# uncbiag/DeepAtlas

Measured on AMD Instinct MI355X. Metric: training volumes/sec at 160x192x160 fp32; Dice vs CPU ref, higher is better.
Workload: dtype f32; 1 GPU; seg-only UNet_light + softmax-Dice + Adam training step, batch 2/GPU, 160x192x160 fp32 (BASELINE configs[1]); global_batch=2, n_classes=32, parallelism=dp1, matrix_precision=fp32_split, hip_graph=False, matrix_arithmetic_bits=22

## Files before the change

### __graft_entry__.py

```python
import os
import subprocess
import sys

ROOT = os.path.dirname(os.path.abspath(__file__))
CSRC = os.path.join(ROOT, 'deepatlas_amd', 'csrc')
LIB = os.path.join(CSRC, 'libdeepatlas_hip.so')
HIP_SOURCES = ['norm_act.hip', 'pool.hip', 'warp.hip', 'losses.hip', 'headdice.hip', 'xent.hip', 'reglosses.hip', 'mi.hip', 'datapath.hip', 'conv3d.hip', 'conv3d_mfma.hip', 'conv3d_flow.hip', 'conv3d_flowmm.hip', 'conv3d_s2.hip', 'conv3d_s2n.hip', 'conv3d_up2.hip', 'deconv.hip', 'pointwise_mfma.hip', 'optim.hip', 'augment.hip', 'regeval.hip', 'jacpen.hip', 'invcons.hip', 'affine.hip', 'fieldinv.hip', 'cc.hip', 'edt.hip', 'intensity.hip']


def _newer(target, deps):
    if not os.path.isfile(target):
        return True
    t = os.path.getmtime(target)
    return any(os.path.getmtime(d) > t for d in deps)


def build(force=False):
    srcs = [os.path.join(CSRC, s) for s in HIP_SOURCES]
    deps = srcs + [os.path.join(CSRC, 'common.h'), os.path.join(CSRC, 'conv3d_internal.h'), os.path.join(CSRC, 'split_f16.h'), os.path.join(CSRC, 'pointwise_internal.h'), os.path.join(CSRC, 'conv3d_wgring.h'), os.path.join(CSRC, 'conv3d_stage.h'), os.path.join(CSRC, 'bspline.h'), os.path.join(CSRC, 'counter_hash.h'),
                   os.path.join(ROOT, 'include', 'deepatlas_hip.h')]
    if force or _newer(LIB, deps):
        hipcc = os.environ.get('HIPCC', '/opt/rocm/bin/hipcc')
        objs = []
        procs = []
        for s in srcs:
            o = s[:-4] + '.o'
            objs.append(o)
            if force or _newer(o, [s] + deps[len(srcs):]):
                procs.append((s, subprocess.Popen([hipcc, '--offload-arch=gfx950', '-O3', '-std=c++17', '-fPIC', '-c', s, '-o', o])))
        for s, p in procs:
            if p.wait() != 0:
                raise RuntimeError('hipcc failed on %s' % s)
        subprocess.check_call([hipcc, '--offload-arch=gfx950', '-shared', '-fPIC'] + objs + ['-o', LIB])
    prim = os.path.join(ROOT, 'oracle', 'prim.c')
    prim_so = os.path.join(ROOT, 'oracle', 'libprim.so')
    if os.path.isfile(prim) and (force or _newer(prim_so, [prim])):
        subprocess.check_call(['gcc', '-O2', '-fPIC', '-shared', '-std=c99', prim, '-lm', '-o', prim_so])
    if ROOT not in sys.path:
        sys.path.insert(0, ROOT)
    import deepatlas_amd
    from deepatlas_amd import _native
    _native.lib()
    return LIB


def build_asan(sources=None, opt='-O1'):
    hipcc = os.environ.get('HIPCC', '/opt/rocm/bin/hipcc')
    out_dir = os.path.join(CSRC, 'asan')
    os.makedirs(out_dir, exist_ok=True)
    names = list(sources) if sources else HIP_SOURCES
    flags = ['--offload-arch=gfx950', '-fsanitize=address', '-fno-gpu-sanitize', '-shared-libsan', '-g', opt, '-std=c++17', '-fPIC']
    procs, objs = [], []
# ... 91 lines not shown
```

### deepatlas_amd/_native.py

```python
import ctypes
import os
from ctypes import c_int, c_float, c_double, c_longlong, c_size_t, c_void_p, c_char_p, POINTER

import torch

_HERE = os.path.dirname(os.path.abspath(__file__))
LIB_PATH = os.environ.get('DA_LIB') or os.path.join(_HERE, 'csrc', 'libdeepatlas_hip.so')

P = c_void_p
I = c_int
F = c_float
LL = c_longlong
SZ = c_size_t
DBL = c_double

SIGNATURES = {
    'da_version': (I, []),
    'da_device_info': (I, [POINTER(c_int), POINTER(c_int), POINTER(c_size_t), c_char_p, I]),
    'da_w_oik_to_tio': (I, [P, P, I, I, I, P]),
    'da_w_tio_to_oik': (I, [P, P, I, I, I, P]),
    'da_w_iok_to_tio': (I, [P, P, I, I, I, P]),
    'da_w_tio_to_iok': (I, [P, P, I, I, I, P]),
    'da_w_iok_flip_to_tio': (I, [P, P, I, I, I, P]),
    'da_w_tio_to_iok_flip': (I, [P, P, I, I, I, P]),
    'da_w_tio_to_oik_acc': (I, [P, P, I, I, I, P]),
    'da_w_tio_to_iok_acc': (I, [P, P, I, I, I, P]),
    'da_w_tio_to_iok_flip_acc': (I, [P, P, I, I, I, P]),
    'da_conv3d_k3_ws_bytes': (SZ, [I, I, I, I, I, I, I]),
    'da_conv3d_k3_pack_bytes': (SZ, [I, I, I, I, I, I]),
    'da_conv3d_k3_dgrad_bst': (I, [P, P, P, I, P, I, I, I, I, I, I, P, P, F, P, I, P, P, SZ, P]),
    'da_conv3d_k3_prepack': (I, [P, I, I, I, I, I, I, I, I, P, SZ, P, SZ, P, P]),
    'da_conv3d_k3_use_prepacked': (None, [P, P, SZ, P, SZ]),
    'da_conv3d_k3_prepack_many': (I, [I, P, P, P, P, P, P, P, P, P, P, P, P, P, P, P]),
    'da_conv3d_k3_fwd': (I, [P, I, P, I, P, P, P, I, I, I, I, I, I, F, P, SZ, P]),
    'da_conv3d_k3_fwd_bnstats': (I, [P, I, P, I, P, P, P, I, I, I, I, I, I, P, I, POINTER(c_int), P, SZ, P]),
    'da_conv3d_k3_dgrad': (I, [P, P, P, I, P, I, I, I, I, I, I, I, P, SZ, P]),
    'da_conv3d_k3_wgrad': (I, [P, I, P, I, P, P, P, I, I, I, I, I, I, P, SZ, P]),
    'da_conv3d_k3_fwd_pro': (I, [P, I, P, P, F, P, I, P, P, F, P, P, P, I, I, I, I, I, F, P, I, POINTER(c_int), P, SZ, P]),
    'da_conv3d_k3_wgrad_pro': (I, [P, I, P, P, F, P, I, P, P, F, P, P, I, I, I, I, I, P, SZ, P]),
    'da_upconv3d_k3_supported': (I, [I, I, I]),
    'da_upconv3d_k3_ws_bytes': (SZ, [I, I, I, I, I, I]),
    'da_upconv3d_k3_fwd': (I, [P, I, P, I, P, P, P, I, I, I, I, I, F, P, SZ, P]),
    'da_upconv3d_k3_dgrad': (I, [P, P, P, I, P, I, I, I, I, I, I, P, SZ, P]),
    'da_upconv3d_k3_wgrad': (I, [P, I, P, I, P, P, I, I, I, I, I, P, SZ, P]),
    'da_set_conv_direct': (I, [I]),
    'da_set_matrix_bf16': (I, [I]),
    'da_set_matrix_mode': (I, [I]),
    'da_pointwise_ws_bytes': (SZ, [I, I, I]),
    'da_conv1x1_fwd': (I, [P, P, P, P, LL, I, I, P, SZ, P]),
    'da_conv1x1_fwd_pro': (I, [P, P, P, F, P, P, P, LL, I, I, P, SZ, P]),
    'da_conv1x1_wgrad_pro': (I, [P, P, P, F, P, P, P, LL, I, I, P, SZ, P]),
    'da_conv1x1_dgrad': (I, [P, P, P, LL, I, I, P, SZ, P]),
    'da_conv1x1_wgrad_ws_bytes': (SZ, [LL, I, I]),
    'da_conv1x1_wgrad': (I, [P, P, P, P, LL, I, I, P, SZ, P]),
    'da_deconv_k2s2_fwd': (I, [P, P, P, P, I, I, I, I, I, I, P, SZ, P]),
    'da_deconv_k2s2_fwd_bnstats': (I, [P, P, P, P, I, I, I, I, I, I, P, I, POINTER(c_int), P, SZ, P]),
    'da_deconv_k2s2_dgrad': (I, [P, P, P, I, I, I, I, I, I, P, SZ, P]),
    'da_deconv_k2s2_bn_bwd_ws_bytes': (SZ, [I, I, I, I, I, I]),
    'da_deconv_k2s2_bn_bwd': (I, [P, P, P, P, P, P, F, P, P, P, P, P, P, P, I, I, I, I, I, I, P, I, P, SZ, P]),
    'da_deconv_k2s2_wgrad_ws_bytes': (SZ, [I, I, I, I, I, I]),
    'da_deconv_k2s2_wgrad': (I, [P, P, P, P, I, I, I, I, I, I, P, SZ, P]),
    'da_bn_ws_bytes': (SZ, [LL, I]),
    'da_bn_train_stats': (I, [P, LL, I, P, P, F, F, P, P, P, P, P, P, P, SZ, P]),
# ... 251 lines not shown
```

### deepatlas_amd/csrc/conv3d_mfma.hip

```cpp
#include "common.h"
#include "conv3d_internal.h"
#include "split_f16.h"

#include "conv3d_stage.h"

namespace {


template <int CK, int NREP, bool MASKED = false, int STATS = 0, bool BF = false, bool PRO = false, bool SP = false, int S2F = 0, bool PAIR = false, bool HB = false>
__global__ void __launch_bounds__(256, 2) conv3_mfma_fwd_kernel(FwdP p) {
    static_assert(!HB || (BF && !SP), "bf16 activation storage: bf16 matrix mode only");
    static_assert(STATS != 2 || (SP && NREP == 1 && !PRO), "BatchNorm-backward sums: the split mode's one-N-tile data gradient");
    static_assert((S2F != 0) == MASKED, "the tap-masked (stride-2) variants and only they address X / dX through the space-to-depth view");
    static_assert(!PAIR || (SP && NREP == 1 && !PRO), "paired staging: split mode, one N-tile, no input prologue");
    static_assert(!SP || (BF && !MASKED && CK == 8), "split mode: dense bf16 K = 32 kernels on 8-channel chunks");
    constexpr int NP = SP ? 2 : 1;
    constexpr bool RAW = HB && BF && !SP && !PRO && !MASKED && S2F == 0;
    extern __shared__ __attribute__((aligned(16))) float lds[];
    constexpr bool K32 = BF && !MASKED;
    using AElem = std::conditional_t<BF, short, float>;
    using Frag = std::conditional_t<SP, f16x8, std::conditional_t<K32, bf16x8, std::conditional_t<BF, s16x4, f32x4>>>;
    constexpr int EB = BF ? 2 : 4;
    constexpr int TZ = 4, HZ = TZ + 2;
    constexpr int NSTEPS = K32 ? (CK == 16 ? 14 : 7) : (27 * CK + 15) / 16;
// ... 1284 lines not shown
                acc[c][d][0] += v.x; acc[c][d][1] += v.y; acc[c][d][2] += v.z; acc[c][d][3] += v.w;
            }
    };
    if (wave >= 2) put(wave - 2);
    __syncthreads();
    if (wave < 2) add(wave);
    __syncthreads();
    if (wave == 1) put(0);
    __syncthreads();
    if (wave == 0) {
        add(0);
        float* part = p.partial + (size_t)slab * p.O;
        const int Cin = p.C1 + p.C2;
        const int co = cg * CG + i;
#pragma unroll
        for (int c = 0; c < 5; ++c)
#pragma unroll
            for (int d = 0; d < 3; ++d)
#pragma unroll
                for (int reg = 0; reg < 4; ++reg) {
                    const int row = 4 * g + reg;
                    const int combo = c < 4 ? 2 * c + (row >> 3) : 8;
                    const int dyt = c < 4 ? d : 2 * d + (row >> 3);
                    const int tap = (combo / 3) * 9 + dyt * 3 + combo % 3, ci = row & 7;
                    if (dyt < 3 && (c < 4 || d < 2) && co < p.Cout) part[((size_t)tap * Cin + cbase + ci) * p.Cout + co] = acc[c][d][reg];
                }
    }
}

#ifndef DA_WG16_ZPAD
#define DA_WG16_ZPAD 4
#endif
#include "conv3d_wgring.h"

__global__ void slab_reduce_kernel(const float* __restrict__ partial, int nparts, int O, float* __restrict__ out) {
    for (int o = blockIdx.x * blockDim.x + threadIdx.x; o < O; o += gridDim.x * blockDim.x) {
        double s = 0.0;
        for (int b = 0; b < nparts; ++b) s += (double)partial[(size_t)b * O + o];
        out[o] = (float)s;
    }
}

struct ScP {
    const float* in1; const float* in2; int C1, C2;
    const float* dy; float* partial;
    int N, D, H, W, Cout; long long nrows;
    const float* dyb; int Cd1;
};

template <int MT, int NT>
__global__ void __launch_bounds__(256) conv3_smallcin_wgrad_kernel(ScP p) {
    __shared__ __attribute__((aligned(16))) float red[MT * NT * 64 * 4];
    const int lane = threadIdx.x & 63;
    const int wave = threadIdx.x >> 6;
    const int i = lane & 15, g = lane >> 4;
    const int Cin = p.C1 + p.C2;
    int dz[MT], dy_[MT], dx[MT], cs[MT], cc[MT]; bool mval[MT]; const float* src[MT];
#pragma unroll
    for (int mt = 0; mt < MT; ++mt) {
        const int m = 16 * mt + i;
        mval[mt] = m < 27 * Cin;
        const int tap = mval[mt] ? m / Cin : 0, ci = mval[mt] ? m % Cin : 0;
        dz[mt] = tap / 9 - 1; dy_[mt] = (tap / 3) % 3 - 1; dx[mt] = tap % 3 - 1;
        if (ci < p.C1) { src[mt] = p.in1; cs[mt] = p.C1; cc[mt] = ci; } else { src[mt] = p.in2; cs[mt] = p.C2; cc[mt] = ci - p.C1; }
    }
    f32x4 acc[MT][NT];
// ... 221 lines not shown
    { static int occ = -1; if (occ < 0) { occ = getenv("DA_OCC") ? 1 : 0; if (occ) { int nb = 0; (void)hipOccupancyMaxActiveBlocksPerMultiprocessor(&nb, kern, 256, shm); fprintf(stderr, "[occ] <%d,%d,M%d,S%d,BF%d,PRO%d,SP%d> lds %zu B -> %d workgroups per CU\n", CK, NREP, (int)MASKED, (int)STATS, (int)BF, (int)PRO, (int)SP, shm, nb); } } }
    if (want) {
        unsigned long long h[6]; (void)hipStreamSynchronize(st); (void)hipMemcpy(h, dclk, 48, hipMemcpyDeviceToHost);
        fprintf(stderr, "[clk] cycles %llu realtime %llu -> %.0f MHz; grid %d x %d: starts span %.1f us, ends span %.1f us, first start -> last end %.1f us\n", h[0], h[1],
                (double)h[0] / (double)h[1] * 100.0, p.nblocks, gy, (h[3] - h[2]) * 0.01, (h[5] - h[4]) * 0.01, (h[5] - h[2]) * 0.01);
        if (getenv("DA_CLK_DUMP")) {
            static unsigned long long rec[2048];
            const int nb = p.nblocks < 1024 ? p.nblocks : 1024;
            (void)hipMemcpy(rec, dclk + 8, (size_t)nb * 16, hipMemcpyDeviceToHost);
            for (int b = 0; b < nb; ++b) fprintf(stderr, "[blk] %d xcc %llu hwid %08llx life_us %.1f\n", b, (rec[2 * b] >> 32) & 15, rec[2 * b] & 0xffffffffull, rec[2 * b + 1] * 0.01);
        }
    }
    return 0;
}

template <int CK, int NREP, unsigned F>
static int launch_fwd_prec(bool bf, bool hb, const FwdP& p, int gy, hipStream_t st) {
    return hb ? launch_fwd_mfma<CK, NREP, F | kHb>(p, gy, st) : bf ? launch_fwd_mfma<CK, NREP, F | kBf16>(p, gy, st) : launch_fwd_mfma<CK, NREP, F>(p, gy, st);
}
template <unsigned F>
static int launch_fwd_dense(int CK, int NREP, bool bf, bool hb, const FwdP& p, int gy, hipStream_t st) {
    if (CK == 16 && NREP == 1) return launch_fwd_prec<16, 1, F>(bf, hb, p, gy, st);
    if (CK == 16 && NREP == 2) return launch_fwd_prec<16, 2, F>(bf, hb, p, gy, st);
    if (CK == 8 && NREP == 1) return launch_fwd_prec<8, 1, F>(bf, hb, p, gy, st);
    if (CK == 8 && NREP == 2) return launch_fwd_prec<8, 2, F>(bf, hb, p, gy, st);
    return DA_ERR_UNSUPPORTED;
}
template <int NREP>
static int launch_fwd_split(bool stats, bool pro, const FwdP& p, int gy, hipStream_t st) {
    return stats ? (pro ? launch_fwd_mfma<8, NREP, kSplit | kStats | kPro>(p, gy, st) : launch_fwd_mfma<8, NREP, kSplit | kStats>(p, gy, st))
                 : (pro ? launch_fwd_mfma<8, NREP, kSplit | kPro>(p, gy, st) : launch_fwd_mfma<8, NREP, kSplit>(p, gy, st));
}

static const int kProMaxC = 2048;
static int pro_identity(const float** ones, const float** zeros) {
    static float* buf = nullptr;
    if (!buf) {
        hipError_t e = hipMalloc(&buf, 2 * kProMaxC * sizeof(float));
        if (e != hipSuccess) return (int)e;
        float* h = (float*)malloc(2 * kProMaxC * sizeof(float));
        for (int i = 0; i < kProMaxC; ++i) { h[i] = 1.f; h[kProMaxC + i] = 0.f; }
        e = hipMemcpy(buf, h, 2 * kProMaxC * sizeof(float), hipMemcpyHostToDevice);
        free(h);
        if (e != hipSuccess) return (int)e;
    }
    *ones = buf; *zeros = buf + kProMaxC;
    return 0;
}

template <typename P>
static int set_prologue(P& p, const DaPro* pro, int C2) {
    p.ps1 = p.pt1 = p.ps2 = p.pt2 = nullptr; p.pslope1 = p.pslope2 = -1.f;
    if (!pro) return 0;
    const float *ones, *zeros;
    if (const int rc = pro_identity(&ones, &zeros)) return rc;
    const float a = pro->s1 ? pro->slope1 : -1.f, b = (C2 > 0 && pro->s2) ? pro->slope2 : -1.f;
    if (a >= 1.f || b >= 1.f) return DA_ERR_UNSUPPORTED;
    p.pslope1 = a < 0.f ? 1.f : a; p.pslope2 = b < 0.f ? 1.f : b;
    p.ps1 = pro->s1 ? pro->s1 : ones; p.pt1 = pro->s1 ? pro->t1 : zeros;
    p.ps2 = (C2 > 0 && pro->s2) ? pro->s2 : ones; p.pt2 = (C2 > 0 && pro->s2) ? pro->t2 : zeros;
    return 0;
}

enum FwdFamily { kFamDense, kFamMasked, kFamSplit, kFamPaired, kFamBst };
struct FwdPlan {
    bool split, bf; int CK, NREP, gy, NTpad;
    int pkmode, NSTEPS;
    size_t pk, tt;
    int ntz, nty, ntx, ntiles, nblocks; FwdFamily family;
};
static int fwd_plan(const ConvGemm& c, int mode, FwdPlan* plan) {
    FwdPlan& q = *plan;
    const int Cin = c.C1 + c.C2;
    q.CK = pick_ck(c.C1, c.C2);
    if (!q.CK) return DA_ERR_UNSUPPORTED;
    if (c.pro && (c.s2d_cin > 0 || c.flipped_tr || Cin > kProMaxC)) return DA_ERR_UNSUPPORTED;
    if (c.s2d_cin > 0 && !c.s2f) return DA_ERR_UNSUPPORTED;
    q.split = mode == 2 && c.s2d_cin == 0;
    q.bf = mode == 1;
    if (q.split) q.CK = 8;
    {
        const int cin = c.C1 > c.C2 ? c.C1 : c.C2, cs = c.Cs1 > c.Cs2 ? c.Cs1 : c.Cs2;
        if ((unsigned long long)c.D * c.H * c.W * 4ull * (unsigned long long)(cin > cs ? cin : cs) >= 0xFFFFFFF0ull) return DA_ERR_UNSUPPORTED;
    }
    const int NT = (c.Cout + 15) / 16;
    q.NREP = pick_nrep(NT);
    if ((q.bf || q.split || c.pro) && q.NREP > 2) q.NREP = 2;
    if (c.s2d_cin > 0 && q.NREP > 2) q.NREP = 2;
    const bool want_bst = c.bst.y != nullptr && q.split && c.stats_partial != nullptr;
    if (want_bst) q.NREP = 1;
    q.ntz = (c.D + 3) / 4; q.nty = (c.H + TY - 1) / TY; q.ntx = (c.W + TX - 1) / TX;
    q.ntiles = c.N * q.ntz * q.nty * q.ntx;
    if (c.s2d_cin == 0 && q.NREP > 1 && !want_bst) {
        const long long tiles = (long long)c.N * q.ntz * q.nty * q.ntx;
        auto cost = [&](int nrep) {
            const int g = (NT + nrep - 1) / nrep;
            long long nb = 512 / g; if (nb < 1) nb = 1; if (nb > tiles) nb = tiles;
            return (double)((tiles + nb - 1) / nb) * nrep * (nrep == 1 ? 1.08 : 1.0);
        };
        if (cost(1) < cost(q.NREP)) q.NREP = 1;
    }
    q.gy = (NT + q.NREP - 1) / q.NREP; q.NTpad = q.gy * q.NREP;
    q.pkmode = q.split ? 3 : q.bf ? (c.s2d_cin > 0 ? 1 : 2) : 0;
    q.NSTEPS = q.pkmode >= 2 ? (q.CK == 16 ? 14 : 7) : (27 * q.CK + 15) / 16;
    q.pk = packed_bytes(Cin, c.Cout, q.CK); q.tt = tile_table_bytes(c.N, c.D, c.H, c.W);
    q.nblocks = 512 / q.gy; if (q.nblocks < 1) q.nblocks = 1; if (q.nblocks > q.ntiles) q.nblocks = q.ntiles;
    if (q.nblocks >= 8) q.nblocks &= ~7;
    if (!q.split) q.family = c.s2d_cin > 0 ? kFamMasked : kFamDense;
    else if (want_bst) q.family = kFamBst;
    else q.family = (q.NREP == 1 && !c.pro && c.C1 % 16 == 0 && c.C2 % 16 == 0) ? kFamPaired : kFamSplit;
    if (q.family == kFamMasked && q.CK != 16) return DA_ERR_UNSUPPORTED;
    if (q.family == kFamBst && (c.pro || c.Cs2 != 0 || q.gy > 2)) return DA_ERR_UNSUPPORTED;
    return 0;
}

static int fwd_launches(const ConvGemm& c, int mode, ConvGemm l[2]) {
    l[0] = c;
    if (!(mode == 2 && c.flipped_tr && c.s2d_cin == 0 && (!c.stats_partial || c.bst.y) && !c.pro && c.Cs1 == 32 && c.Cs2 == 16 && c.Cout == 48 &&
          pick_ck(c.C1, c.C2) != 0)) return 1;
    l[0].out2 = nullptr; l[0].Cs2 = 0; l[0].Cout = 32; l[0].CoutW = 48; l[0].pack = ConvPack{{c.pack.buf[0], nullptr}, {c.pack.bytes[0], 0}};
    l[1] = l[0];
    l[1].bias = c.bias ? c.bias + 32 : nullptr; l[1].out1 = c.out2; l[1].Cs1 = 16; l[1].Cout = 16; l[1].cout0 = 32;
    l[1].stats_partial = nullptr; l[1].stats_nparts = nullptr; l[1].bst = ConvBst{}; l[1].pack = ConvPack{{c.pack.buf[1], nullptr}, {c.pack.bytes[1], 0}};
    return 2;
}

static PackJob pack_job(const ConvGemm& c, const FwdPlan& q, char* base) {
    return PackJob{c.w_tio, reinterpret_cast<unsigned short*>(base), reinterpret_cast<int*>(base + q.pk - da_align(kWexpInts * sizeof(int))), reinterpret_cast<int4*>(base + q.pk),
                   c.C1 + c.C2, c.Cout, q.NTpad, c.flipped_tr, q.ntiles, q.ntx, q.nty, q.ntz, c.cout0, c.CoutW ? c.CoutW : c.Cout};
}
static void launch_split_pack(const PackJob& j, hipStream_t st) {
    hipLaunchKernelGGL(pack_split_weights_kernel, dim3(j.Cin / 8, 8), dim3(256), 0, st, j.w, j.wp, j.wexp, j.Cin, j.Cout, j.NTpad, j.flipped, j.tiles, j.ntiles, j.ntx, j.nty, j.ntz, j.cout0, j.CoutW);
}

struct Handover { const float* w; ConvPack pack; };
static thread_local Handover g_handover = {nullptr, {}};
static ConvPack take_handover(const float* w_tio) {
    const Handover h = g_handover;
    g_handover = Handover{nullptr, {}};
    return h.w == w_tio ? h.pack : ConvPack{};
}

static int conv3_mfma_launch(const ConvGemm& c) {
    FwdPlan q;
    if (const int rc = fwd_plan(c, da_matrix_mode(), &q)) return rc;
    const int Cin = c.C1 + c.C2, CK = q.CK, NREP = q.NREP, gy = q.gy;
    const bool bf = q.bf, hb = c.act_bf16 != 0, stats = c.stats_partial != nullptr, pro = c.pro != nullptr;
    hipStream_t st = c.st;
    const bool kept = q.split && c.pack.buf[0] && c.pack.bytes[0] >= q.pk + q.tt;
    if (!kept && c.ws_bytes < q.pk + q.tt) return DA_ERR_WS_SMALL;
    if (q.split && Cin / 8 > kWexpInts) return DA_ERR_UNSUPPORTED;
    const PackJob j = pack_job(c, q, kept ? reinterpret_cast<char*>(const_cast<void*>(c.pack.buf[0])) : reinterpret_cast<char*>(c.ws));
    const long long total = (long long)(Cin / CK) * q.NSTEPS * q.NTpad * 256;
    if (!q.split)
        hipLaunchKernelGGL(pack_fwd_weights_kernel, dim3(da_grid(total > q.ntiles ? total : q.ntiles, 256, 1024)), dim3(256), 0, st, c.w_tio, reinterpret_cast<float*>(j.wp), Cin, c.Cout, CK, q.NSTEPS, q.NTpad,
                           c.flipped_tr, total, q.pkmode, j.tiles, q.ntiles, q.ntx, q.nty, q.ntz, j.cout0, j.CoutW);
    else if (!kept) launch_split_pack(j, st);
    DA_LAUNCH_CHECK();
    FwdP p;
    const bool bst = q.family == kFamBst;
    p.bst_y = bst ? c.bst.y : nullptr; p.bst_par = bst ? c.bst.par : nullptr; p.bst_slope = bst ? c.bst.slope : -1.f;
    p.tiles = j.tiles; p.wp = reinterpret_cast<float*>(j.wp); p.wexp = j.wexp;
    p.in1 = c.in1; p.in2 = c.in2; p.C1 = c.C1; p.C2 = c.C2; p.bias = c.bias;
    p.out1 = c.out1; p.out2 = c.out2; p.Cs1 = c.Cs1; p.Cs2 = c.Cs2;
    p.N = c.N; p.D = c.D; p.H = c.H; p.W = c.W; p.Cout = c.Cout; p.NT = q.NTpad;
    p.ntz = q.ntz; p.nty = q.nty; p.ntx = q.ntx; p.ntiles = q.ntiles; p.nblocks = q.nblocks; p.slope = c.slope;
    p.maskmode = q.family != kFamMasked ? 0 : c.flipped_tr ? 2 : 1;
    if (p.maskmode == 1) da_s2d_masks(p.masks, Cin / 16, 16, c.s2d_cin, 0);
    if (p.maskmode == 2) da_s2d_masks(p.masks, gy, NREP * 16, c.s2d_cin, 1);
    { static int abl = -1; if (abl < 0) { const char* e = getenv("DA_ABLATE"); abl = e ? atoi(e) : 0; } p.ablate = abl; }
    p.s2in = S2dSrc{0, 0, 0, 0}; p.s2out = S2dSrc{0, 0, 0, 0};
    if (c.s2d_cin > 0) (c.flipped_tr ? p.s2out : p.s2in) = S2dSrc{c.s2d_cin, c.s2f->D0, c.s2f->H0, c.s2f->W0};
    p.stats_partial = c.stats_partial;
    if (c.stats_nparts) *c.stats_nparts = 0;
    if (const int rc = set_prologue(p, c.pro, c.C2)) return rc;
    if (q.split) {
        if (stats && c.stats_nparts) *c.stats_nparts = p.nblocks;
        if (bst) return launch_fwd_mfma<8, 1, kSplit | kBst>(p, gy, st);
        if (q.family == kFamPaired) return stats ? launch_fwd_mfma<8, 1, kSplit | kStats | kPair>(p, gy, st) : launch_fwd_mfma<8, 1, kSplit | kPair>(p, gy, st);
        return NREP == 1 ? launch_fwd_split<1>(stats, pro, p, gy, st) : launch_fwd_split<2>(stats, pro, p, gy, st);
    }
    if (stats && p.maskmode == 0 && NREP <= 2) {
        if (c.stats_nparts) *c.stats_nparts = p.nblocks;
        return pro ? launch_fwd_dense<kStats | kPro>(CK, NREP, bf, hb, p, gy, st) : launch_fwd_dense<kStats>(CK, NREP, bf, hb, p, gy, st);
    }
    if (pro) return launch_fwd_dense<kPro>(CK, NREP, bf, hb, p, gy, st);
    if (p.maskmode != 0) {
        if (NREP == 1) return p.maskmode == 1 ? launch_fwd_prec<16, 1, kS2dIn>(bf, hb, p, gy, st) : launch_fwd_prec<16, 1, kD2sOut>(bf, hb, p, gy, st);
        if (NREP == 2) return p.maskmode == 1 ? launch_fwd_prec<16, 2, kS2dIn>(bf, hb, p, gy, st) : launch_fwd_prec<16, 2, kD2sOut>(bf, hb, p, gy, st);
        return DA_ERR_UNSUPPORTED;
    }
    if (NREP == 3 && !bf) {
        if (CK == 16) return launch_fwd_mfma<16, 3>(p, gy, st);
        if (CK == 8) return launch_fwd_mfma<8, 3>(p, gy, st);
    }
    return launch_fwd_dense<0>(CK, NREP, bf, hb, p, gy, st);
}

int da_conv3_mfma_fwd(const ConvGemm& call) {
    if (call.act_bf16 && da_matrix_mode() != 1) return DA_ERR_UNSUPPORTED;
    ConvGemm c = call, l[2];
    c.pack = take_handover(c.w_tio);
    const int n = fwd_launches(c, da_matrix_mode(), l);
    for (int i = 0; i < n; ++i)
        if (const int rc = conv3_mfma_launch(l[i])) return rc;
    return 0;
}

static int g_matrix_mode = -1;
int da_matrix_mode() {
// ... 238 lines not shown
    if (rc) return rc;
    return da_reduce_partials(p.partial, q.nslabs, p.O, dw_tio, st);
}

extern "C" size_t da_conv3d_k3_pack_bytes(int N, int D, int H, int W, int Cin, int Cout) {
    if (Cin % 8 != 0 && Cout % 8 != 0) return 0;
    size_t a = Cin % 8 == 0 ? packed_bytes(Cin, Cout, 8) : 0;
    if (Cout % 8 == 0) { const size_t b = packed_bytes(Cout, Cin, 8); if (b > a) a = b; }
    return a + tile_table_bytes(N, D, H, W);
}
static int prepack_jobs(const float* w_tio, int C1, int C2, int Cout, int dgrad, int N, int D, int H, int W, void* b0, size_t n0, void* b1, size_t n1, PackJob jobs[2], int* njobs) {
    *njobs = 0;
    if (!w_tio || !b0 || C1 <= 0 || C2 < 0 || Cout <= 0 || N <= 0) return DA_ERR_BADARG;
    if (da_matrix_mode() != 2) return 0;
    const int Cin = C1 + C2;
    if (!dgrad ? !da_conv3_mfma_fwd_supported(C1, C2, Cout, 1) : !da_conv3_mfma_fwd_supported(Cout, 0, Cin, 1, C1, C2)) return 0;
    ConvGemm c = {}, l[2];
    c.w_tio = w_tio; c.flipped_tr = dgrad; c.N = N; c.D = D; c.H = H; c.W = W; c.slope = -1.f;
    if (!dgrad) { c.C1 = C1; c.C2 = C2; c.Cs1 = Cout; c.Cout = Cout; }
    else { c.C1 = Cout; c.Cs1 = C1; c.Cs2 = C2; c.Cout = Cin; }
    const int n = fwd_launches(c, 2, l);
    void* const buf[2] = {b0, b1}; const size_t bytes[2] = {n0, b1 ? n1 : 0};
    for (int i = 0; i < n; ++i) {
        FwdPlan q;
        int rc = fwd_plan(l[i], 2, &q);
        if (!rc && (!buf[i] || bytes[i] < q.pk + q.tt)) rc = DA_ERR_WS_SMALL;
        if (!rc && (l[i].C1 + l[i].C2) / 8 > kWexpInts) rc = DA_ERR_UNSUPPORTED;
        if (rc) return rc == DA_ERR_UNSUPPORTED ? 0 : rc;
        jobs[i] = pack_job(l[i], q, reinterpret_cast<char*>(buf[i]));
    }
    *njobs = n;
    return 0;
}
extern "C" int da_conv3d_k3_prepack(const float* w_tio, int C1, int C2, int Cout, int dgrad, int N, int D, int H, int W,
                                    void* b0, size_t n0, void* b1, size_t n1, int* used, void* stream) {
    if (used) *used = 0;
    PackJob jobs[2]; int n = 0;
    if (const int rc = prepack_jobs(w_tio, C1, C2, Cout, dgrad, N, D, H, W, b0, n0, b1, n1, jobs, &n)) return rc;
    for (int i = 0; i < n; ++i) { launch_split_pack(jobs[i], (hipStream_t)stream); DA_LAUNCH_CHECK(); }
    if (used) *used = n;
    return 0;
}
extern "C" void da_conv3d_k3_use_prepacked(const float* w_tio, const void* b0, size_t n0, const void* b1, size_t n1) {
    g_handover = (w_tio && b0) ? Handover{w_tio, ConvPack{{b0, b1}, {n0, b1 ? n1 : 0}}} : Handover{nullptr, {}};
}

extern "C" int da_conv3d_k3_prepack_many(int n, const float* const* w_tio, const int* C1, const int* C2, const int* Cout, const int* dgrad,
                                         const int* N, const int* D, const int* H, const int* W,
                                         void* const* b0, const size_t* n0, void* const* b1, const size_t* n1, int* used, void* stream) {
    if (n <= 0) return 0;
    if (!w_tio || !C1 || !C2 || !Cout || !dgrad || !N || !D || !H || !W || !b0 || !n0 || !b1 || !n1 || !used) return DA_ERR_BADARG;
    PackJobs jobs; int njobs = 0;
    auto flush = [&]() -> int {
        if (njobs == 0) return 0;
        int gx = 1;
        for (int k = 0; k < njobs; ++k) if (jobs.j[k].Cin / 8 > gx) gx = jobs.j[k].Cin / 8;
        hipLaunchKernelGGL(pack_split_weights_many_kernel, dim3(gx, 8, njobs), dim3(256), 0, (hipStream_t)stream, jobs);
        njobs = 0;
        DA_LAUNCH_CHECK();
        return 0;
    };
    int rc = 0;
    for (int i = 0; i < n && !rc; ++i) {
        if (njobs + 2 > kPackJobsMax && (rc = flush())) break;
        rc = prepack_jobs(w_tio[i], C1[i], C2[i], Cout[i], dgrad[i], N[i], D[i], H[i], W[i], b0[i], n0[i], b1[i], n1[i], &jobs.j[njobs], &used[i]);
        njobs += used[i];
// ... 23 lines not shown
```

### include/deepatlas_hip.h

```cpp
#ifndef DEEPATLAS_HIP_H
#define DEEPATLAS_HIP_H

#include <stddef.h>
#include <stdint.h>

#ifdef __cplusplus
extern "C" {
#endif

#define DA_ERR_BADARG   (-1)
#define DA_ERR_WS_SMALL (-2)
#define DA_ERR_UNSUPPORTED (-3)

int  da_version(void);
int  da_device_info(int* cu_count, int* wave_size, size_t* hbm_bytes, char* arch, int arch_len);

int da_w_oik_to_tio(const float* w_oik, float* w_tio, int Cout, int Cin, int K3, void* stream);
int da_w_tio_to_oik(const float* w_tio, float* w_oik, int Cout, int Cin, int K3, void* stream);
int da_w_iok_to_tio(const float* w_iok, float* w_tio, int Cin, int Cout, int K3, void* stream);
int da_w_tio_to_iok(const float* w_tio, float* w_iok, int Cin, int Cout, int K3, void* stream);
int da_w_iok_flip_to_tio(const float* w_iok, float* w_tio, int Cin, int Cout, int K3, void* stream);
int da_w_tio_to_iok_flip(const float* w_tio, float* w_iok, int Cin, int Cout, int K3, void* stream);
int da_w_tio_to_oik_acc(const float* w_tio, float* w_oik, int Cout, int Cin, int K3, void* stream);
int da_w_tio_to_iok_acc(const float* w_tio, float* w_iok, int Cin, int Cout, int K3, void* stream);
// ... 159 lines not shown
                                float* dlogits, int N, int D, int H, int W, int C, void* stream);
size_t da_warp_bwd_dsrc_det_ws_bytes(int N, int D, int H, int W, int C);
int da_warp_bwd_dsrc_det(const float* dout, const float* disp, float* d_src, int N, int D, int H, int W, int C,
                         void* ws, size_t ws_bytes, void* stream);

size_t da_dice_ws_bytes(int N, long long V, int C);
int da_dice_fwd(const float* src, const void* labels, int label_bytes, const float* soft_target,
                int N, long long V, int C, int softmax, int weight_type, int no_bg, float eps,
                float* loss, float* coef, void* ws, size_t ws_bytes, void* stream);
int da_dice_bwd(const float* src, const void* labels, int label_bytes, const float* soft_target,
                const float* coef, const float* dloss, float* d_src,
                int N, long long V, int C, int softmax, void* stream);
int da_softmax_fwd(const float* x, float* y, long long M, int C, void* stream);
int da_softmax_bwd(const float* dy, const float* y, float* dx, long long M, int C, void* stream);
int da_one_hot(const void* labels, int label_bytes, float* out, long long M, int C, void* stream);

size_t da_head_dice_ws_bytes(int N, long long V, int Cin, int C);
int da_head_dice_fwd(const float* x, const float* pro_scale, const float* pro_shift, float pro_slope,
                     const float* w_io, const float* bias, const void* labels, int label_bytes,
                     int N, long long V, int Cin, int C, int weight_type, int no_bg, float eps,
                     float* loss, float* coef, void* ws, size_t ws_bytes, void* stream);
int da_head_dice_bwd(const float* x, const float* pro_scale, const float* pro_shift, float pro_slope,
                     const float* w_io, const float* bias, const void* labels, int label_bytes,
                     const float* coef, const float* dloss, float* dx, float* dw_io, float* dbias,
                     int N, long long V, int Cin, int C, void* ws, size_t ws_bytes, void* stream);
int da_head_dice_bwd_bst(const float* x, const float* pro_scale, const float* pro_shift, float pro_slope, const float* pro_mean,
                         const float* w_io, const float* bias, const void* labels, int label_bytes,
                         const float* coef, const float* dloss, float* dx, float* dw_io, float* dbias,
                         int N, long long V, int Cin, int C, double* bst, int bst_cap, int* bst_n, void* ws, size_t ws_bytes, void* stream);

int da_conv3d_k3_dgrad_bst(const float* dy, const float* w_tio, float* dx1, int C1, float* dx2, int C2, int N, int D, int H, int W, int Cout,
                           const float* y, const float* stats4, float slope, double* bst, int bst_cap, int* bst_n,
                           void* ws, size_t ws_bytes, void* stream);

size_t da_conv3d_k3_pack_bytes(int N, int D, int H, int W, int Cin, int Cout);
int da_conv3d_k3_prepack(const float* w_tio, int C1, int C2, int Cout, int dgrad, int N, int D, int H, int W,
                         void* b0, size_t n0, void* b1, size_t n1, int* used, void* stream);
void da_conv3d_k3_use_prepacked(const float* w_tio, const void* b0, size_t n0, const void* b1, size_t n1);
int da_conv3d_k3_prepack_many(int n, const float* const* w_tio, const int* C1, const int* C2, const int* Cout, const int* dgrad,
                              const int* N, const int* D, const int* H, const int* W,
                              void* const* b0, const size_t* n0, void* const* b1, const size_t* n1, int* used, void* stream);

size_t da_ncc_ws_bytes(int N, long long V);
int da_ncc_fwd(const float* x, const float* y, int N, long long V, float* loss, double* stats ,
               void* ws, size_t ws_bytes, void* stream);
int da_ncc_bwd(const float* x, const float* y, const double* stats, const float* dloss,
               float* dx, float* dy, int N, long long V, void* stream);

size_t da_bending_ws_bytes(int N, int D, int H, int W);
int da_bending_fwd(const float* disp, int N, int D, int H, int W, const float* spacing3, int normalize, int norm,
                   float* loss, void* ws, size_t ws_bytes, void* stream);
int da_bending_bwd(const float* disp, const float* dloss, float* d_disp, int N, int D, int H, int W,
                   const float* spacing3, int normalize, int norm, void* stream);

size_t da_xent_ws_bytes(void);
int da_xent_fwd(const float* logits, const void* labels, int label_bytes, const float* soft_target, const float* alpha,
                long long M, int C, int mode, int softmax, float gamma, long long ignore_index, int reduction,
                float* loss, float* denom, void* ws, size_t ws_bytes, void* stream);
int da_xent_bwd(const float* logits, const void* labels, int label_bytes, const float* soft_target, const float* alpha,
                const float* dloss, const float* denom, float* dlogits, long long M, int C, int mode, int softmax, float gamma,
                long long ignore_index, void* stream);

int da_conv_k2s2_fwd(const float* x, const float* w_tio, const float* bias, float* y,
                     int N, int D, int H, int W, int Cin, int Cout, void* ws, size_t ws_bytes, void* stream);
int da_conv_k2s2_dgrad(const float* dy, const float* w_tio, float* dx,
                       int N, int D, int H, int W, int Cin, int Cout, void* ws, size_t ws_bytes, void* stream);
// ... 214 lines not shown
```

Measured before the change: 99.79 volumes/s.

## Add z-streaming ring-buffered split-fp16 forward conv kernel for 8/16-channel layers

Adds a new forward 3x3x3 conv kernel for layers with 8 or 16 input channels and at most 16 outputs. Each block keeps the full reduction depth and weights resident in LDS and walks consecutive z-tiles through a 10-slot ring of input planes, prefetching the next planes while the MFMA work for the current tile runs. It also fuses the optional stats and backward-stat epilogues. The goal is to avoid reloading halo planes and weights for every tile and to hide global-load latency behind compute. The price is a new, complex code path with shared exponent scaling that must match across tiles, extra LDS pressure, and a persistent-grid schedule.

Result: no change. 100.3 volumes/s, median of 6 (+0.6%).

```diff
diff --git a/__graft_entry__.py b/__graft_entry__.py
--- a/__graft_entry__.py
+++ b/__graft_entry__.py
@@ -17,7 +17,7 @@
 
 def build(force=False):
     srcs = [os.path.join(CSRC, s) for s in HIP_SOURCES]
-    deps = srcs + [os.path.join(CSRC, 'common.h'), os.path.join(CSRC, 'conv3d_internal.h'), os.path.join(CSRC, 'split_f16.h'), os.path.join(CSRC, 'pointwise_internal.h'), os.path.join(CSRC, 'conv3d_wgring.h'), os.path.join(CSRC, 'conv3d_stage.h'), os.path.join(CSRC, 'bspline.h'), os.path.join(CSRC, 'counter_hash.h'),
+    deps = srcs + [os.path.join(CSRC, 'common.h'), os.path.join(CSRC, 'conv3d_internal.h'), os.path.join(CSRC, 'split_f16.h'), os.path.join(CSRC, 'pointwise_internal.h'), os.path.join(CSRC, 'conv3d_wgring.h'), os.path.join(CSRC, 'conv3d_fwdring.h'), os.path.join(CSRC, 'conv3d_stage.h'), os.path.join(CSRC, 'bspline.h'), os.path.join(CSRC, 'counter_hash.h'),
                    os.path.join(ROOT, 'include', 'deepatlas_hip.h')]
     if force or _newer(LIB, deps):
         hipcc = os.environ.get('HIPCC', '/opt/rocm/bin/hipcc')
diff --git a/deepatlas_amd/_native.py b/deepatlas_amd/_native.py
--- a/deepatlas_amd/_native.py
+++ b/deepatlas_amd/_native.py
@@ -29,6 +29,7 @@
     'da_conv3d_k3_ws_bytes': (SZ, [I, I, I, I, I, I, I]),
     'da_conv3d_k3_pack_bytes': (SZ, [I, I, I, I, I, I]),
     'da_conv3d_k3_dgrad_bst': (I, [P, P, P, I, P, I, I, I, I, I, I, P, P, F, P, I, P, P, SZ, P]),
+    'da_conv3d_k3_ring_tiles': (I, [I, I, I, I, I, I, P]),
     'da_conv3d_k3_prepack': (I, [P, I, I, I, I, I, I, I, I, P, SZ, P, SZ, P, P]),
     'da_conv3d_k3_use_prepacked': (None, [P, P, SZ, P, SZ]),
     'da_conv3d_k3_prepack_many': (I, [I, P, P, P, P, P, P, P, P, P, P, P, P, P, P, P]),
diff --git a/deepatlas_amd/csrc/conv3d_fwdring.h b/deepatlas_amd/csrc/conv3d_fwdring.h
--- /dev/null
+++ b/deepatlas_amd/csrc/conv3d_fwdring.h
@@ -0,0 +1,291 @@
+template <int CIN, int STATS>
+__global__ void __launch_bounds__(CIN == 16 ? 512 : 256, CIN == 16 ? 1 : 2) conv3_split_fwdring_kernel(FwdP p) {
+    static_assert(CIN == 8 || CIN == 16, "the whole reduction depth is resident: 8 or 16 input channels");
+    using Frag = f16x8;
+    extern __shared__ __attribute__((aligned(16))) float lds[];
+    constexpr int NW = CIN == 16 ? 8 : 4, NTH = NW * 64, NCH = CIN / 8, Q = CIN / 4;
+    constexpr int RPW = 32 / NW;
+    constexpr int RPB = STATS == 2 ? 2 : 4;
+    constexpr int PV = HY * HX, SLOT_E = PV * 8, NSLOT = 10;
+    constexpr int CH_E = NSLOT * SLOT_E, PLANE_E = NCH * CH_E;
+    constexpr int HSQ = 2 * PV * Q;
+    constexpr int HS = (HSQ + NTH - 1) / NTH;
+    constexpr int NS = NCH * 7;
+    constexpr unsigned OOR = 0xFFFFFFFFu;
+    const short* ldsh = reinterpret_cast<const short*>(lds);
+    const short* ldsw = ldsh + 2 * PLANE_E;
+    float* smax = lds + PLANE_E + NS * 512;
+    double* sred = reinterpret_cast<double*>(smax + 64);
+    const int lane = threadIdx.x & 63;
+    const int wave = __builtin_amdgcn_readfirstlane((int)(threadIdx.x >> 6));
+    const int i = lane & 15, g = lane >> 4;
+    const int zs = NW == 8 ? wave >> 1 : wave, r0 = NW == 8 ? (wave & 1) * RPW : 0;
+    const int Cs = p.C1;
+
+    const int c4 = (int)threadIdx.x % Q;
+    unsigned pk[HS]; int vo[HS], ldsq[HS];
+#pragma unroll
+    for (int it = 0; it < HS; ++it) {
+        const int idx = (int)threadIdx.x + it * NTH, hv = idx / Q;
+        const int hz = hv / PV, rem = hv - hz * PV, hy = rem / HX, hx = rem - hy * HX;
+        const bool ok = idx < HSQ;
+        pk[it] = ok ? ((unsigned)hz << 16 | (unsigned)hy << 8 | (unsigned)hx) : 0xFFFF0000u;
+        vo[it] = ok ? (hz * p.H + hy) * p.W + hx : 0;
+        ldsq[it] = ok ? (c4 >> 1) * (CH_E / 4) + (hz * PV + rem) * 2 + (c4 & 1) : 0;
+    }
+    const bool smallA = (long long)2 * p.H * p.W < (1ll << 24) && (long long)Cs * 4 < (1ll << 24);
+    const unsigned Cs4 = (unsigned)Cs * 4u, cofs4 = (unsigned)(c4 * 4) * 4u;
+    const bool has_pro = p.ps1 != nullptr;
+    float4 psc = make_float4(1.f, 1.f, 1.f, 1.f), psf = make_float4(0.f, 0.f, 0.f, 0.f);
+    if (has_pro) { psc = *reinterpret_cast<const float4*>(p.ps1 + c4 * 4); psf = *reinterpret_cast<const float4*>(p.pt1 + c4 * 4); }
+    const float pslope = p.pslope1;
+
+    float4 pre[3][HS];
+    unsigned vm = 0;
+    auto issue_pair = [&](auto HC, int n, int zf, int y0, int x0, bool valid) {
+        constexpr int h = decltype(HC)::value;
+        const __amdgpu_buffer_rsrc_t rs = da_rsrc_n<false>(p.in1, n, (long long)p.D * p.H * p.W * Cs);
+        const bool interior = smallA && valid && zf >= 0 && zf + 2 <= p.D && y0 >= 1 && y0 + HY - 2 < p.H && x0 >= 1 && x0 + HX - 2 < p.W;
+        const unsigned base = (unsigned)((zf * p.H + (y0 - 1)) * p.W + (x0 - 1)) * Cs4 + cofs4;
+        vm &= ~(255u << (8 * h));
+#pragma unroll
+        for (int it = 0; it < HS; ++it) {
+            const int hz = (int)(pk[it] >> 16), hy = (int)((pk[it] >> 8) & 255u), hx = (int)(pk[it] & 255u);
+            unsigned so;
+            if (interior) so = ((it + 1) * NTH <= HSQ || hz < 2) ? __umul24((unsigned)vo[it], Cs4) + base : OOR;
+            else {
+                const int z = zf + hz, y = y0 - 1 + hy, x = x0 - 1 + hx;
+                const bool inb = valid && hz < 2 && (unsigned)z < (unsigned)p.D && (unsigned)y < (unsigned)p.H && (unsigned)x < (unsigned)p.W;
+                so = inb ? (unsigned)((z * p.H + y) * p.W + x) * Cs4 + cofs4 : OOR;
+            }
+            pre[h][it] = da_buf_load4(rs, so);
+            vm |= (so != OOR ? 1u : 0u) << (8 * h + it);
+        }
+    };
+    auto finish_pair = [&](auto HC, float* slot) {
+        constexpr int h = decltype(HC)::value;
+        if (has_pro) stage_pro_apply<0, HS>(pre[h], vm >> (8 * h), psc, psf, pslope);
+        const float m = da_wave_max_nonneg(stage_absmax<HS>(pre[h]));
+        if (lane == 0) slot[h * NW + wave] = m;
+    };
+    auto read_exp = [&](const float* s) -> int {
+        float m;
+        if constexpr (NW == 8) {
+            const float4 a = *reinterpret_cast<const float4*>(s), b = *reinterpret_cast<const float4*>(s + 4);
+            m = fmaxf(fmaxf(fmaxf(a.x, a.y), fmaxf(a.z, a.w)), fmaxf(fmaxf(b.x, b.y), fmaxf(b.z, b.w)));
+        } else {
+            const float4 a = *reinterpret_cast<const float4*>(s);
+            m = fmaxf(fmaxf(a.x, a.y), fmaxf(a.z, a.w));
+        }
+        return da_scale_exp(__int_as_float(__builtin_amdgcn_readfirstlane(__float_as_int(m))));
+    };
+    auto write_pair = [&](auto HC, int rp, float sa) {
+        constexpr int h = decltype(HC)::value;
+        uint2* L = reinterpret_cast<uint2*>(lds) + rp * (2 * SLOT_E / 4);
+#pragma unroll
+        for (int it = 0; it < HS; ++it)
+            if ((it + 1) * NTH <= HSQ || (pk[it] >> 16) < 2u) da_split_store4(pre[h][it], sa, L + ldsq[it], PLANE_E / 4);
+    };
+
+    int tapz[7], tapo[7];
+#pragma unroll
+    for (int s = 0; s < 7; ++s) {
+        int tap = 4 * s + g; tap = tap > 26 ? 26 : tap;
+        tapz[s] = zs + tap / 9;
+        tapo[s] = ((r0 + (tap / 3) % 3) * HX + i + tap % 3) * 8;
+    }
+    {
+        const __amdgpu_buffer_rsrc_t rsw = __builtin_amdgcn_make_buffer_rsrc((void*)p.wp, 0, (unsigned)(NS * p.NT * 2048), 0x00020000);
+        uint4* W = reinterpret_cast<uint4*>(lds + PLANE_E);
+        for (int u = threadIdx.x; u < NS * 128; u += NTH) {
+            const int sp = u >> 6;
+            W[u] = __builtin_bit_cast(uint4, __builtin_amdgcn_raw_buffer_load_b128(rsw, (unsigned)(u & 63) * 16u, (unsigned)(((sp >> 1) * p.NT * 2 + (sp & 1)) * 1024), 0));
+        }
+    }
+    auto wb = [&](int gs, int pl) -> Frag { return *reinterpret_cast<const Frag*>(ldsw + (gs * 2 + pl) * 512 + lane * 8); };
+    float bvv[4];
+#pragma unroll
+    for (int j = 0; j < 4; ++j) { const int co = 4 * g + j; bvv[j] = (p.bias && co < p.Cout) ? p.bias[co] : 0.f; }
+    const bool cq_ok = 4 * g + 3 < p.Cout;
+    const int ew0 = p.wexp[0], ew1 = NCH == 2 ? p.wexp[1] : 0;
+    float4 bmu = make_float4(0.f, 0.f, 0.f, 0.f), bsc = bmu, bsf = bmu;
+    if constexpr (STATS == 2) {
+        const __amdgpu_buffer_rsrc_t rp = da_rsrc(p.bst_par, (unsigned)(4 * p.Cs1 * 4));
+        const unsigned po = cq_ok ? (unsigned)(4 * g * 4) : OOR;
+        bmu = da_buf_load4(rp, po);
+        bsc = da_buf_load4(rp, po == OOR ? po : po + (unsigned)(2 * p.Cs1 * 4));
+        bsf = da_buf_load4(rp, po == OOR ? po : po + (unsigned)(3 * p.Cs1 * 4));
+    }
+    double ds1[STATS ? 4 : 1], ds2[STATS ? 4 : 1];
+#pragma unroll
+    for (int j = 0; j < (STATS ? 4 : 1); ++j) { ds1[j] = 0.0; ds2[j] = 0.0; }
+
+    const int G = gridDim.x, tps = (p.ntiles + G - 1) / G;
+    const int ridx = (G % 8 == 0) ? ((int)blockIdx.x % 8) * (G / 8) + (int)blockIdx.x / 8 : (int)blockIdx.x;
+    const int lo = ridx * tps, hi = min(lo + tps, p.ntiles);
+    int pos = lo, par = 0;
+#pragma unroll 1
+    while (pos < hi) {
+        const int tz0 = pos % p.ntz, col = pos / p.ntz, tx0 = col % p.ntx, rr = col / p.ntx;
+        const int n = rr / p.nty, z0 = 4 * tz0, y0 = (rr % p.nty) * TY, x0 = tx0 * TX;
+        const int nrun = min(hi - pos, p.ntz - tz0);
+        issue_pair(IntC<0>{}, n, z0 - 1, y0, x0, true);
+        issue_pair(IntC<1>{}, n, z0 + 1, y0, x0, true);
+        issue_pair(IntC<2>{}, n, z0 + 3, y0, x0, true);
+        finish_pair(IntC<0>{}, smax + par * 3 * NW);
+        finish_pair(IntC<1>{}, smax + par * 3 * NW);
+        finish_pair(IntC<2>{}, smax + par * 3 * NW);
+        __syncthreads();
+        int e_sh = read_exp(smax + (par * 3 + 2) * NW);
+        const int ea = min(min(read_exp(smax + (par * 3 + 0) * NW), read_exp(smax + (par * 3 + 1) * NW)), e_sh);
+        const int E0 = ea + ew0, E1 = NCH == 2 ? da_split_cap(ea + ew1, false, E0) : E0;
+        const float sa = (NCH == 2 && (c4 >> 1)) ? da_pow2(E1 - ew1) : da_pow2(ea);
+        const float f01 = da_acc_factor(E1 - E0);
+        float inv1, inv2; da_unscale_factors(E1, inv1, inv2);
+        write_pair(IntC<0>{}, 0, sa);
+        write_pair(IntC<1>{}, 1, sa);
+        write_pair(IntC<2>{}, 2, sa);
+        par ^= 1;
+        int P = 0, t = 0;
+        bool have_next = nrun > 1;
+        issue_pair(IntC<1>{}, n, z0 + 5, y0, x0, have_next);
+        issue_pair(IntC<2>{}, n, z0 + 7, y0, x0, have_next);
+        finish_pair(IntC<1>{}, smax + par * 3 * NW);
+        finish_pair(IntC<2>{}, smax + par * 3 * NW);
+        __syncthreads();
+#pragma unroll 1
+        for (;;) {
+            const int zt = z0 + 4 * t;
+            const int eN0 = read_exp(smax + (par * 3 + 1) * NW), eN1 = read_exp(smax + (par * 3 + 2) * NW);
+            const int e_new = min(eN0, eN1);
+            const bool conv = have_next && ea <= e_new && ea >= min(e_sh, e_new) - 3;
+            const bool have_next2 = conv && t + 2 < nrun;
+            if (conv) {
+                const int N0 = P + 3 >= 5 ? P - 2 : P + 3, N1 = P + 4 >= 5 ? P - 1 : P + 4;
+                write_pair(IntC<1>{}, N0, sa);
+                write_pair(IntC<2>{}, N1, sa);
+                e_sh = eN1;
+            }
+            issue_pair(IntC<1>{}, n, zt + 9, y0, x0, have_next2);
+            issue_pair(IntC<2>{}, n, zt + 11, y0, x0, have_next2);
+
+            int aoff[7];
+#pragma unroll
+            for (int s = 0; s < 7; ++s) { int sl = 2 * P + tapz[s]; sl = sl >= NSLOT ? sl - NSLOT : sl; aoff[s] = sl * SLOT_E + tapo[s]; }
+            f32x4 acc[RPW];
+#pragma unroll
+            for (int r = 0; r < RPW; ++r) acc[r] = (f32x4){0.f, 0.f, 0.f, 0.f};
+            auto aptr = [&](int gs) -> const short* { return ldsh + (gs / 7) * CH_E + aoff[gs % 7]; };
+            float4 yq[STATS == 2 ? RPW : 1];
+            const int z = zt + zs, x = x0 + i;
+            const bool cok = cq_ok && z < p.D && x < p.W;
+            Frag AC[2][RPB], bq[2][2];
+            bq[0][0] = wb(0, 0); bq[0][1] = wb(0, 1);
+            {
+                const short* ap = aptr(0);
+#pragma unroll
+                for (int pl = 0; pl < 2; ++pl)
+#pragma unroll
+                    for (int q = 0; q < RPB; ++q) AC[pl][q] = *reinterpret_cast<const Frag*>(ap + pl * PLANE_E + q * (HX * 8));
+            }
+#pragma unroll
+            for (int gs = 0; gs < NS; ++gs) {
+                if (gs + 1 < NS) { bq[(gs + 1) & 1][0] = wb(gs + 1, 0); bq[(gs + 1) & 1][1] = wb(gs + 1, 1); }
+                if constexpr (STATS == 2) {
+                    if (gs == NS - 1) {
+                        const __amdgpu_buffer_rsrc_t ry = da_rsrc_n<false>(p.bst_y, n, (long long)p.D * p.H * p.W * p.Cs1);
+#pragma unroll
+                        for (int r = 0; r < RPW; ++r) {
+                            const int y = y0 + r0 + r;
+                            const unsigned off = ((unsigned)((z * p.H + y) * p.W + x) * (unsigned)p.Cs1 + (unsigned)(4 * g)) * 4u;
+                            yq[r] = da_buf_load4(ry, (cok && y < p.H) ? off : OOR);
+                        }
+                    }
+                }
+                if (NCH == 2 && gs == 7 && E1 != E0) {
+#pragma unroll
+                    for (int r = 0; r < RPW; ++r) acc[r] = acc[r] * f01;
+                }
+                const short* ap = aptr(gs);
+                const short* anx = gs + 1 < NS ? aptr(gs + 1) : ap;
+#pragma unroll
+                for (int qd = 0; qd < RPW / RPB; ++qd) {
+                    Frag AN[2][RPB];
+                    const short* src = (qd + 1 < RPW / RPB) ? ap + (RPB * qd + RPB) * (HX * 8) : anx;
+#pragma unroll
+                    for (int pl = 0; pl < 2; ++pl)
+#pragma unroll
+                        for (int q = 0; q < RPB; ++q) AN[pl][q] = *reinterpret_cast<const Frag*>(src + pl * PLANE_E + q * (HX * 8));
+#pragma unroll
+                    for (int pr = 0; pr < 3; ++pr)
+#pragma unroll
+                        for (int q = 0; q < RPB; ++q) {
+                            acc[RPB * qd + q] = __builtin_amdgcn_mfma_f32_16x16x32_f16(bq[gs & 1][kSplitPB[pr]], AC[kSplitPA[pr]][q], acc[RPB * qd + q], 0, 0, 0);
+                        }
+                    __builtin_amdgcn_sched_barrier(0);
+#pragma unroll
+                    for (int pl = 0; pl < 2; ++pl)
+#pragma unroll
+                        for (int q = 0; q < RPB; ++q) AC[pl][q] = AN[pl][q];
+                }
+            }
+            {
+                float st1[STATS ? 4 : 1], st2[STATS ? 4 : 1];
+#pragma unroll
+                for (int j = 0; j < (STATS ? 4 : 1); ++j) { st1[j] = 0.f; st2[j] = 0.f; }
+                const __amdgpu_buffer_rsrc_t ro = da_rsrc_n<false>(p.out1, n, (long long)p.D * p.H * p.W * p.Cs1);
+#pragma unroll
+                for (int r = 0; r < RPW; ++r) {
+                    const int y = y0 + r0 + r;
+                    const float v0 = acc[r][0] * inv1 * inv2 + bvv[0], v1 = acc[r][1] * inv1 * inv2 + bvv[1];
+                    const float v2 = acc[r][2] * inv1 * inv2 + bvv[2], v3 = acc[r][3] * inv1 * inv2 + bvv[3];
+                    if constexpr (STATS == 2) {
+                        const float m = (cok && y < p.H) ? 1.f : 0.f;
+                        const float4 yv = yq[r];
+                        const float d0 = m * v0 * da_act_grad(yv.x * bsc.x + bsf.x, p.bst_slope), d1 = m * v1 * da_act_grad(yv.y * bsc.y + bsf.y, p.bst_slope);
+                        const float d2 = m * v2 * da_act_grad(yv.z * bsc.z + bsf.z, p.bst_slope), d3 = m * v3 * da_act_grad(yv.w * bsc.w + bsf.w, p.bst_slope);
+                        st1[0] += d0; st1[1] += d1; st1[2] += d2; st1[3] += d3;
+                        st2[0] += d0 * (yv.x - bmu.x); st2[1] += d1 * (yv.y - bmu.y); st2[2] += d2 * (yv.z - bmu.z); st2[3] += d3 * (yv.w - bmu.w);
+                    } else if constexpr (STATS == 1) {
+                        const float m = (cok && y < p.H) ? 1.f : 0.f;
+                        st1[0] += m * v0; st1[1] += m * v1; st1[2] += m * v2; st1[3] += m * v3;
+                        st2[0] += m * v0 * v0; st2[1] += m * v1 * v1; st2[2] += m * v2 * v2; st2[3] += m * v3 * v3;
+                    }
+                    const unsigned off = ((unsigned)((z * p.H + y) * p.W + x) * (unsigned)p.Cs1 + (unsigned)(4 * g)) * 4u;
+                    da_buf_store4(ro, (cok && y < p.H) ? off : OOR, (f32x4){da_act(v0, p.slope), da_act(v1, p.slope), da_act(v2, p.slope), da_act(v3, p.slope)});
+                }
+                if constexpr (STATS != 0) {
+#pragma unroll
+                    for (int j = 0; j < 4; ++j) { ds1[j] += (double)st1[j]; ds2[j] += (double)st2[j]; }
+                }
+            }
+            if (have_next2) {
+                finish_pair(IntC<1>{}, smax + (par ^ 1) * 3 * NW);
+                finish_pair(IntC<2>{}, smax + (par ^ 1) * 3 * NW);
+            }
+            __syncthreads();
+            if (!conv) break;
+            P = P + 2 >= 5 ? P - 3 : P + 2; t += 1; have_next = have_next2; par ^= 1;
+        }
+        pos += t + 1;
+    }
+    if constexpr (STATS != 0) {
+#pragma unroll
+        for (int j = 0; j < 4; ++j) {
+            double a = ds1[j], b = ds2[j];
+            a += __shfl_xor(a, 1); b += __shfl_xor(b, 1);
+            a += __shfl_xor(a, 2); b += __shfl_xor(b, 2);
+            a += __shfl_xor(a, 4); b += __shfl_xor(b, 4);
+            a += __shfl_xor(a, 8); b += __shfl_xor(b, 8);
+            if (i == 0) { sred[(wave * 2 + 0) * 16 + 4 * g + j] = a; sred[(wave * 2 + 1) * 16 + 4 * g + j] = b; }
+        }
+        __syncthreads();
+        if ((int)threadIdx.x < 16 && (int)threadIdx.x < p.Cout) {
+            double a = 0.0, b = 0.0;
+#pragma unroll
+            for (int w = 0; w < NW; ++w) { a += sred[(w * 2 + 0) * 16 + threadIdx.x]; b += sred[(w * 2 + 1) * 16 + threadIdx.x]; }
+            p.stats_partial[((size_t)blockIdx.x * 2 + 0) * p.Cout + threadIdx.x] = a;
+            p.stats_partial[((size_t)blockIdx.x * 2 + 1) * p.Cout + threadIdx.x] = b;
+        }
+    }
+}
diff --git a/deepatlas_amd/csrc/conv3d_mfma.hip b/deepatlas_amd/csrc/conv3d_mfma.hip
--- a/deepatlas_amd/csrc/conv3d_mfma.hip
+++ b/deepatlas_amd/csrc/conv3d_mfma.hip
@@ -1340,6 +1340,7 @@
 #define DA_WG16_ZPAD 4
 #endif
 #include "conv3d_wgring.h"
+#include "conv3d_fwdring.h"
 
 __global__ void slab_reduce_kernel(const float* __restrict__ partial, int nparts, int O, float* __restrict__ out) {
     for (int o = blockIdx.x * blockDim.x + threadIdx.x; o < O; o += gridDim.x * blockDim.x) {
@@ -1627,6 +1628,17 @@
                  : (pro ? launch_fwd_mfma<8, NREP, kSplit | kPro>(p, gy, st) : launch_fwd_mfma<8, NREP, kSplit>(p, gy, st));
 }
 
+template <int CIN, int STATS>
+static int launch_fwd_ring_one(const FwdP& p, hipStream_t st) {
+    constexpr int NW = CIN == 16 ? 8 : 4;
+    const size_t shm = (size_t)(CIN / 8) * 10 * HY * HX * 8 * 2 * 2 + (size_t)(CIN / 8) * 7 * 2048 + 64 * sizeof(float) + (STATS ? (size_t)NW * 32 * sizeof(double) : 0);
+    return da_launch_lds<conv3_split_fwdring_kernel<CIN, STATS>>(dim3(p.nblocks), dim3(NW * 64), shm, st, p);
+}
+static int launch_fwd_ring(int Cin, int stats, const FwdP& p, hipStream_t st) {
+    if (Cin == 16) return stats == 2 ? launch_fwd_ring_one<16, 2>(p, st) : stats == 1 ? launch_fwd_ring_one<16, 1>(p, st) : launch_fwd_ring_one<16, 0>(p, st);
+    return stats == 2 ? launch_fwd_ring_one<8, 2>(p, st) : stats == 1 ? launch_fwd_ring_one<8, 1>(p, st) : launch_fwd_ring_one<8, 0>(p, st);
+}
+
 static const int kProMaxC = 2048;
 static int pro_identity(const float** ones, const float** zeros) {
     static float* buf = nullptr;
@@ -1657,7 +1669,10 @@
     return 0;
 }
 
-enum FwdFamily { kFamDense, kFamMasked, kFamSplit, kFamPaired, kFamBst };
+enum FwdFamily { kFamDense, kFamMasked, kFamSplit, kFamPaired, kFamBst, kFamRing };
+static bool fwd_ring_shape(const ConvGemm& c) {
+    return c.s2d_cin == 0 && c.C2 == 0 && (c.C1 == 8 || c.C1 == 16) && c.Cout <= 16 && c.Cs2 == 0 && c.CoutW == 0 && c.D >= 5;
+}
 struct FwdPlan {
     bool split, bf; int CK, NREP, gy, NTpad;
     int pkmode, NSTEPS;
@@ -1706,6 +1721,12 @@
     else q.family = (q.NREP == 1 && !c.pro && c.C1 % 16 == 0 && c.C2 % 16 == 0) ? kFamPaired : kFamSplit;
     if (q.family == kFamMasked && q.CK != 16) return DA_ERR_UNSUPPORTED;
     if (q.family == kFamBst && (c.pro || c.Cs2 != 0 || q.gy > 2)) return DA_ERR_UNSUPPORTED;
+    if (q.split && fwd_ring_shape(c)) {
+        q.family = kFamRing;
+        int g = c.C1 == 16 ? 256 : 512;
+        if (g > q.ntiles / 8) g = (q.ntiles / 8) & ~7;
+        q.nblocks = g >= 8 ? g : (q.ntiles >= 16 ? 8 : q.ntiles);
+    }
     return 0;
 }
 
@@ -1753,7 +1774,8 @@
     else if (!kept) launch_split_pack(j, st);
     DA_LAUNCH_CHECK();
     FwdP p;
-    const bool bst = q.family == kFamBst;
+    const bool want_bst = c.bst.y != nullptr && q.split && stats;
+    const bool bst = q.family == kFamBst || (q.family == kFamRing && want_bst);
     p.bst_y = bst ? c.bst.y : nullptr; p.bst_par = bst ? c.bst.par : nullptr; p.bst_slope = bst ? c.bst.slope : -1.f;
     p.tiles = j.tiles; p.wp = reinterpret_cast<float*>(j.wp); p.wexp = j.wexp;
     p.in1 = c.in1; p.in2 = c.in2; p.C1 = c.C1; p.C2 = c.C2; p.bias = c.bias;
@@ -1771,6 +1793,7 @@
     if (const int rc = set_prologue(p, c.pro, c.C2)) return rc;
     if (q.split) {
         if (stats && c.stats_nparts) *c.stats_nparts = p.nblocks;
+        if (q.family == kFamRing) return launch_fwd_ring(c.C1, want_bst ? 2 : stats ? 1 : 0, p, st);
         if (bst) return launch_fwd_mfma<8, 1, kSplit | kBst>(p, gy, st);
         if (q.family == kFamPaired) return stats ? launch_fwd_mfma<8, 1, kSplit | kStats | kPair>(p, gy, st) : launch_fwd_mfma<8, 1, kSplit | kPair>(p, gy, st);
         return NREP == 1 ? launch_fwd_split<1>(stats, pro, p, gy, st) : launch_fwd_split<2>(stats, pro, p, gy, st);
@@ -2075,6 +2098,14 @@
     *njobs = n;
     return 0;
 }
+extern "C" int da_conv3d_k3_ring_tiles(int N, int D, int H, int W, int C1, int Cout, int* ntz) {
+    ConvGemm c = {};
+    c.C1 = C1; c.Cs1 = Cout; c.Cout = Cout; c.N = N; c.D = D; c.H = H; c.W = W;
+    FwdPlan q;
+    if (N <= 0 || !da_conv3_mfma_fwd_supported(C1, 0, Cout, 1) || fwd_plan(c, 2, &q) || q.family != kFamRing) return 0;
+    if (ntz) *ntz = q.ntz;
+    return (int)da_cdiv(q.ntiles, q.nblocks);
+}
 extern "C" int da_conv3d_k3_prepack(const float* w_tio, int C1, int C2, int Cout, int dgrad, int N, int D, int H, int W,
                                     void* b0, size_t n0, void* b1, size_t n1, int* used, void* stream) {
     if (used) *used = 0;
diff --git a/include/deepatlas_hip.h b/include/deepatlas_hip.h
--- a/include/deepatlas_hip.h
+++ b/include/deepatlas_hip.h
@@ -215,6 +215,8 @@
 int da_conv3d_k3_dgrad_bst(const float* dy, const float* w_tio, float* dx1, int C1, float* dx2, int C2, int N, int D, int H, int W, int Cout,
                            const float* y, const float* stats4, float slope, double* bst, int bst_cap, int* bst_n,
                            void* ws, size_t ws_bytes, void* stream);
+
+int da_conv3d_k3_ring_tiles(int N, int D, int H, int W, int C1, int Cout, int* ntz);
 
 size_t da_conv3d_k3_pack_bytes(int N, int D, int H, int W, int Cin, int Cout);
 int da_conv3d_k3_prepack(const float* w_tio, int C1, int C2, int Cout, int dgrad, int N, int D, int H, int W,
```
